# Vasilispapg/CVML-GoalNet

Hardware: AMD Instinct MI355X
Metric: training clips/sec at batch 64, 16-frame 224² clips; logit MAE vs CPU ref (higher is better)
Workload: dtype f32; 1 GPU; AVM train step (forward + broadcast-MSE + backward + fused Adam), 64 clips x 16 frames = 1024 frames of 3x224x224 + 30x30 MFCC per GPU; dropout live (device masks), BatchNorm train mode; frames_per_gpu=1024, h=224, w=224, parallelism=dp1, ddp_semantics=local BN + local MSE per rank, gradient mean (standard DDP), params=1286754369

## Files before the change

### cvml_goalnet_amd/_lib.py

```python
from __future__ import annotations

import ctypes
import os
from ctypes import c_char_p, c_double, c_float, c_int, c_int64, c_size_t, c_uint32, c_uint64, c_void_p

_HERE = os.path.dirname(os.path.abspath(__file__))
LIB_PATH = os.environ.get("GOALNET_LIB_PATH") or os.path.join(_HERE, "libgoalnet_hip.so")
ABI_VERSION = 7
STAT_PARTS = 1024
ADAM_RANGES_MAX = 32

P = c_void_p


class RowCopy(ctypes.Structure):
    _fields_ = [("src", c_void_p), ("dst", c_void_p), ("row_bytes", c_int64), ("nrows", c_int), ("gather", c_int), ("cursor", c_void_p),
                ("cursor_bias", c_int64)]


class AdamRange(ctypes.Structure):
    _fields_ = [("begin", c_int64), ("count", c_int64), ("skipped", c_int64)]


PROTOTYPES = {
# ... 55 lines not shown
    "goalnet_split_padded": (c_int, [c_int, P, P, P, P, P, c_int, c_int, c_int, c_int, P]),
    "goalnet_split_rows": (c_int, [c_int, P, c_int64, P, P, c_int, P, P, c_int64, c_int64, P]),
    "goalnet_conv3x3_fwd_split": (c_int, [c_int, P, P, P, c_int, P, c_int, c_int, c_int, c_int, c_int, P, P]),
    "goalnet_conv3x3_wgrad_split_ws_bytes": (c_size_t, [c_int, c_int, c_int, c_int, c_int, c_int]),
    "goalnet_conv3x3_wgrad_split": (c_int, [c_int, P, P, P, P, c_size_t, c_int, c_int, c_int, c_int, c_int, P, P]),
    "goalnet_linear_split_ok": (c_int, [c_int, c_int, c_int64, c_int]),
    "goalnet_linear_fwd_split_ws_bytes": (c_size_t, [c_int, c_int, c_int64, c_int]),
    "goalnet_linear_fwd_split": (c_int, [c_int, P, P, P, c_int, P, c_int64, P, c_int64, P, c_int64, c_int, c_int64, c_int, P, c_size_t, P, P]),
    "goalnet_linear_bwd_dx_split": (c_int, [c_int, P, P, P, c_int64, c_int, c_int64, c_int, P, P]),
    "goalnet_linear_bwd_dw_split": (c_int, [c_int, P, P, P, c_int, c_int64, c_int, P, P]),
    "goalnet_linear_bwd_dx_bf16": (c_int, [P, c_int64, P, P, c_int64, P, c_int64, c_int, c_int64, c_int, c_int, P]),
    "goalnet_linear_bwd_dx_bf16_o16_ok": (c_int, [c_int, c_int64, c_int]),
    "goalnet_linear_bwd_dx_bf16_o16": (c_int, [P, c_int64, P, P, c_int64, c_int, c_int64, c_int, c_int, P]),
    "goalnet_conv3x3_fwd_bf16p_o16_ok": (c_int, [c_int, c_int, c_int, c_int, c_int]),
    "goalnet_conv3x3_fwd_bf16p_o16": (c_int, [P, P, P, c_int, P, c_int, c_int, c_int, c_int, c_int, c_int, P]),
    "goalnet_linear_bwd_dw_bf16": (c_int, [P, c_int64, P, c_int64, P, c_int, c_int64, c_int, c_int, P]),
    "goalnet_linear_fwd_ws_bytes": (c_size_t, [c_int, c_int64, c_int]),
    "goalnet_linear_fwd": (c_int, [P, c_int64, P, P, c_int, P, P, c_int, P, c_int64, P, c_int64, P, c_int64,
                                   c_int, c_int64, c_int, P, c_size_t, P]),
    "goalnet_linear_bwd_dx": (c_int, [P, c_int64, P, P, c_int64, P, c_int64, c_int, c_int64, c_int, P]),
    "goalnet_linear_bwd_dw": (c_int, [P, c_int64, P, c_int64, P, P, c_int, P, P, c_int, c_int64, c_int, P]),
    "goalnet_linear_bwd_dw_adam": (c_int, [P, c_int64, P, c_int64, P, P, c_int, P, P, P, P, c_int, c_int64, c_int,
                                           c_double, c_double, c_double, c_double, P, c_int64, c_float, P]),
    "goalnet_colsum": (c_int, [P, c_int64, c_int, c_int, P, P]),
    "goalnet_mul": (c_int, [P, c_int64, P, c_int64, P, c_int64, c_int, c_int, P]),
    "goalnet_conv1d_fwd": (c_int, [P, P, P, c_int, P, c_int, c_int, c_int, c_int, c_int, c_int, P]),
    "goalnet_conv1d_bwd_ws_bytes": (c_size_t, [c_int, c_int, c_int]),
    "goalnet_conv1d_bwd": (c_int, [P, P, P, P, P, P, c_int, c_int, c_int, c_int, c_int, c_int, P, c_size_t, P]),
    "goalnet_conv1d_bwd_small": (c_int, [P, P, P, P, P, P, P, c_int, c_int, c_int, c_int, c_int, c_int, P]),
    "goalnet_relu_bwd": (c_int, [P, P, P, c_int64, P]),
    "goalnet_mlp_blocks": (c_int, []),
    "goalnet_mlp_fwd": (c_int, [P, c_int64, c_int, P, P, P, P, P, P, P, P, P, P, P, c_int, P, P]),
    "goalnet_mlp_bwd_ws_bytes": (c_size_t, [c_int]),
    "goalnet_mlp_bwd": (c_int, [P, P, P, c_int64, P, c_int64, P, P, P, P, c_int64, P, c_int, c_int, c_int, P, c_size_t, P, P]),
    "goalnet_head_fwd": (c_int, [P, c_int64, P, P, P, P, c_int, c_int, P]),
    "goalnet_head_bwd": (c_int, [P, P, P, c_int64, P, P, c_int64, P, c_int64, P, P, c_int, c_int, P]),
    "goalnet_mse_bcast": (c_int, [P, P, c_int, P, P, P]),
    "goalnet_cubic_resample": (c_int, [P, P, P, c_int64, c_int, c_int, P]),
    "goalnet_logmel_slots": (c_int, [P, P, P, c_int, c_int, P, P, P, P, P, P, P, P]),
    "goalnet_mfcc_from_logmel": (c_int, [P, P, c_int, c_int, P, P, P, P, c_int, c_int, c_double, P]),
    "goalnet_cls_head_fwd": (c_int, [P, c_int64, P, P, P, P, c_int, c_int, c_int, P]),
    "goalnet_cross_entropy": (c_int, [P, P, P, P, c_int, c_int, P]),
    "goalnet_cls_head_bwd": (c_int, [P, P, P, c_int64, P, P, c_int64, P, c_int64, P, P, c_int, c_int, c_int, P]),
    "goalnet_argmax_plus1": (c_int, [P, P, c_int, c_int, P]),
    "goalnet_adam_step": (c_int, [P, P, P, P, c_int64, c_double, c_double, c_double, c_double, c_int, c_float, P]),
    "goalnet_counter_add": (c_int, [P, c_int64, P]),
# ... 67 lines not shown
```

### cvml_goalnet_amd/avm.py

```python
from __future__ import annotations

import math
import os
from typing import List, Optional

import torch
import torch.nn as nn
from torch.nn.parameter import UninitializedParameter

from . import ops
from ._lib import GoalnetError
from .synth import BASE_SEED, DROP_P, TID_DROP

F32 = torch.float32
BN_EPS = 1e-5
BN_MOMENTUM = 0.1
_ALIGN = 64


class _LazyFlags:

    def requires_grad_(self, requires_grad: bool = True):
        for p in self.parameters():
            p.requires_grad = requires_grad
# ... 48 lines not shown
            return r, None
        ev = torch.cuda.Event()
        ev.record(self.side)
        return r, ev

    @staticmethod
    def wait(ev):
        if ev is not None:
            torch.cuda.current_stream().wait_event(ev)

    def join(self):
        if self.enabled and self.forked:
            torch.cuda.current_stream().wait_stream(self.side)
            self.forked = False
        self.keep.clear()


class _Bwd:

    def __init__(self, model, train, fork):
        self.model, self.train, self.fork = model, train, fork
        self.scratch = {}
        self.dbias = {}
        self.T = train.__contains__

    def any_T(self, *layers):
        return any(f"{layer}.{leaf}" in self.train for layer in layers for leaf in ("weight", "bias"))

    def G(self, name):
        m = self.model
        if name in self.train:
            return m._gflat(name)
        s = m.spec(name)
        if s.kind in ("ohwi", "lin5") and name != "visbl.conv1.weight":
            raise GoalnetError(f"a backward that does not train {name} asked for its gradient")
        t = self.scratch.get(name)
        if t is None:
            t = self.scratch[name] = torch.empty(s.numel, dtype=F32, device=m._device)
        return t


class _Spec:
    __slots__ = ("name", "kind", "shape", "numel", "offset", "fan_in")

    def __init__(self, name, kind, shape, fan_in):
        self.name, self.kind, self.shape, self.fan_in = name, kind, tuple(shape), fan_in
# ... 16 lines not shown
    return out


EPI_FUSE_MIN_ROWS = 256
EPI_FUSE_SKINNY_ROWS = 16


def epi_fuse_pieces(env):
    if env is None or env in ("", "1"):
        return frozenset("a")
    if env == "0":
        return frozenset()
    return frozenset(ch for ch in env.lower() if ch in "a")


def epi_fuse_dw_adam(n, *, plain, synced, precision, train_w5, shadowed, inspected, forced, pieces):
    if forced is False or "a" not in pieces:
        return False
    if inspected and forced is not True:
        return False
    if not (plain and not synced and precision == "fp32" and train_w5 and not shadowed):
        return False
    if n <= EPI_FUSE_SKINNY_ROWS:
        return False
    return forced is True or n >= EPI_FUSE_MIN_ROWS


class AVM(_LazyFlags, nn.Module):
    def __init__(self, audio_included, device=None, seed: Optional[int] = None, precision: str = "fp32", head: str = "regression",
                 num_classes: int = 5):
        super().__init__()
        self.audio_included = audio_included
        if head not in ("regression", "classifier"):
            raise ValueError("head must be 'regression' (the reference's live code) or 'classifier' (its commented-out variant)")
        if not 2 <= num_classes <= 8:
            raise ValueError("num_classes must be in 2..8")
        self.head = head
        self.num_classes = num_classes if head == "classifier" else 1
        if precision not in ("fp32", "bf16", "fp16", "bf16x6", "fp16x3"):
            raise ValueError("precision must be 'fp32' (the reference's arithmetic), 'bf16x6' / 'fp16x3' (fp32 operands as bf16 triples / scaled "
                             "fp16 pairs on the 16-bit MFMA: fp32-grade), 'bf16' or 'fp16' (16-bit MFMA contractions)")
        self._loss_scale, self._loss_scale_user = 1.0, False
        self._loss_scale_backoff = 0
        self._skipped_seen = 0
        self.precision = precision
        self._guard = None
# ... 30 lines not shown
        self._sat_out = {}
        self._bwd_frozen = frozenset()
        self._fp16_frozen = None
        self._arena_grad_scale = 1.0
        self._w5b, self._w5b_version = None, None
        self._load_count = 0
        self._state = None
        self._materialized = False
        self.grad_sync = None
        self.stat_sync = None
        self.grad_bf16 = os.environ.get("GOALNET_DZ16", "1") != "0"
        self.act_bf16 = os.environ.get("GOALNET_P16", "1") != "0"
        env = os.environ.get
        self.x6_off = env("GOALNET_X6_OFF") == "1"
        self.x6_linear5 = env("GOALNET_X6_LINEAR5", "1") != "0"
        self.x3_wgrad2 = env("GOALNET_X3_WGRAD2", "1") != "0"
        self.x3_dgrad2 = env("GOALNET_X3_DGRAD2", "1") != "0"
        self.mlp_fused = env("GOALNET_MLP_FUSED", "1") != "0"
        self.small_bn = env("GOALNET_SMALL_BN", "1") != "0"
        self.force_bf5 = env("GOALNET_FORCE_BF5") == "1"
        self.overlap_pair = env("GOALNET_OVERLAP_PAIR", "1") != "0"
        self.epi_fuse = None
        self.epi_fused_dw = 0
        self.keep_ctx = False
        self.last_ctx = None
        self.last_used_w5b = False
        self._side_stream = None
        self.overlap_rows = int(os.environ.get("GOALNET_OVERLAP_ROWS", "64"))
        _ol = os.environ.get("GOALNET_OVERLAP_LARGE")
        self.overlap_large = _ol == "1"
        self.overlap_auto = _ol is None
        self.time_labels = None
        self.kernel_events = None

    @property
    def precision(self) -> str:
        return self._precision

    @precision.setter
    def precision(self, value: str):
        if value not in ("fp32", "bf16", "fp16", "bf16x6", "fp16x3"):
            raise ValueError("precision must be 'fp32', 'bf16x6', 'fp16x3', 'bf16' or 'fp16'")
        self._precision = value
        self._half = value in ("bf16", "fp16")
        self._parts = {"bf16x6": 3, "fp16x3": 2}.get(value, 0)
        self._x6 = self._parts > 0
# ... 334 lines not shown
        return ops.split_padded(self._parts, x, scale, shift, self._padbuf(key, n, h, w, self._parts * c), n, h, w, c, amax=am), am

    def _split_mat(self, x2d, rows, c, scale=None, shift=None, bnC=0):
        am = self._amax_of(x2d, rows, c, scale=scale, shift=shift, bnC=bnC)
        return ops.split_rows(self._parts, x2d, torch.empty(rows * self._parts * c, dtype=self._h16, device=x2d.device), rows, c,
                              scale=scale, shift=shift, bnC=bnC, amax=am), am

    def _x6_linear5(self, n, k5):
        return self._x6 and ops.linear_split_ok(self._parts, n, k5, 512) and not self.x6_off and self.x6_linear5

    def _mlp_fused(self, n):
        return n <= 16 and self.head == "regression" and self.mlp_fused

    def _bf5(self, n):
        return self._half and (n > 16 or self.force_bf5)

    def _pair(self, n):
        return self._large_overlap(n) and self.overlap_pair

    def _small_bn(self, a, b, n, hc, wc, c):
        return (a.dtype == F32 and b.dtype == F32 and self.stat_sync is None and c <= 512 and n * hc * wc * c <= ops.SMALL_BN_ELEMS
                and self.small_bn)

    def _bn_block(self, y, n, hc, wc, c, i, save, p16=False):
        dev = self._device
        assert p16 or y.dtype == F32
        p = torch.empty(n, hc - 2, wc - 2, c, dtype=self._h16 if p16 else F32, device=dev)
        idx = torch.empty(n, hc - 2, wc - 2, c, dtype=torch.uint8, device=dev) if save else None
        bn = getattr(self.visbl, f"bnorm{i}")
        st = torch.empty(4, c, dtype=F32, device=dev)
        count = n * (hc - 2) * (wc - 2)
        if not self.training:
            ops.pool_bn_eval_fwd(y, p, idx, self._pflat(f"visbl.bnorm{i}.weight"), self._pflat(f"visbl.bnorm{i}.bias"),
                                 bn.running_mean, bn.running_var, BN_EPS, st, n, hc, wc, c)
            return p, idx, st
        if self._small_bn(y, p, n, hc, wc, c):
            ops.pool_bn_fwd_small(y, p, idx, self._pflat(f"visbl.bnorm{i}.weight"), self._pflat(f"visbl.bnorm{i}.bias"),
                                  bn.running_mean, bn.running_var, BN_MOMENTUM, BN_EPS, st, n, hc, wc, c)
            bn.num_batches_tracked += 1
            return p, idx, st
        partials = torch.empty(ops.stat_parts(8 * n) * 2 * c, dtype=torch.float64, device=dev)
        ops.pool_bnstats_fwd(y, p, idx, partials, n, hc, wc, c)
        if self.stat_sync is not None:
            partials, count = self._global_sums(partials, 2 * c), count * self.stat_sync.world
        ops.bn_finalize(partials, self._pflat(f"visbl.bnorm{i}.weight"), self._pflat(f"visbl.bnorm{i}.bias"),
                        bn.running_mean, bn.running_var, BN_MOMENTUM, BN_EPS, count, c,
# ... 125 lines not shown
            x = hs[4]
        for li, (key, width) in enumerate(() if fused_mlp else (("0", 512), ("3", 512), ("6", 256), ("9", 128))):
            hnext = torch.empty(n, width, dtype=F32, device=dev)
            m = torch.empty(n, width, dtype=F32, device=dev) if save else None
            ops.linear_fwd(x, P(f"fusion.{key}.weight"), P(f"fusion.{key}.bias"), hnext, relu=True,
                           dropmask=masks[1 + li], mult_out=m)
            hs.append(hnext); ms.append(m)
            x = hnext
        if self.head == "classifier":
            logit = torch.empty(n, self.num_classes, dtype=F32, device=dev)
            out = torch.empty(n, self.num_classes, dtype=F32, device=dev)
            ops.cls_head_fwd(x, P("fusion.12.weight"), P("fusion.12.bias"), logit, out)
        elif not fused_mlp:
            logit = torch.empty(n, dtype=F32, device=dev)
            out = torch.empty(n, dtype=F32, device=dev)
            ops.head_fwd(x, P("fusion.12.weight"), P("fusion.12.bias"), logit, out)
        if save:
            ctx.update(p1=p1, idx1=idx1, st1=st1, p2=p2, idx2=idx2, st2=st2, p3=p3, idx3=idx3, st3=st3,
                       a1=a1, a2=a2, hs=hs, ms=ms, logit=logit, out=out, l1=l1, l2=l2)
        self.last_logit = logit
        self.last_features = cat
        return out, ctx

    def _block_bwd(self, bwd, dbn, ctx, i, n, hc, wc, c):
        dev, G, bias = self._device, bwd.G, bwd.T(f"visbl.conv{i}.bias")
        p, idx, st = ctx[f"p{i}"], ctx[f"idx{i}"], ctx[f"st{i}"]
        npix = n * (hc - 2) * (wc - 2)
        small = self._small_bn(dbn, p, n, hc, wc, c) and not (self._half and i > 1)
        frozen = ctx["eval"]
        if small:
            coef3 = torch.empty(3 * c, dtype=F32, device=dev)
            (ops.bn_bwd_reduce_small_eval if frozen else ops.bn_bwd_reduce_small)(
                dbn, p, st[0], st[1], self._pflat(f"visbl.bnorm{i}.weight"), G(f"visbl.bnorm{i}.weight"), G(f"visbl.bnorm{i}.bias"),
                coef3, n, hc, wc, c)
            dy = torch.empty(n, hc, wc, c, dtype=F32, device=dev)
            dparts = torch.empty(ops.stat_parts(8 * n) * c, dtype=torch.float64, device=dev)
            ops.bnpool_bwd(dbn, p, idx, coef3, dy, dparts, n, hc, wc, c)
            if i > 1 and bias:
                bwd.dbias[i] = (dparts, c)
            return dy
        coef3 = torch.empty(3 * c, dtype=F32, device=dev)
        partials = torch.empty(ops.stat_parts(npix // 64) * 2 * c, dtype=torch.float64, device=dev)
        ops.bn_bwd_reduce(dbn, p, st[0], st[1], partials, npix, c)
        if frozen:
            ops.bn_bwd_finalize_eval(partials, self._pflat(f"visbl.bnorm{i}.weight"), st[1], c,
                                     G(f"visbl.bnorm{i}.weight"), G(f"visbl.bnorm{i}.bias"), coef3)
        else:
            ops.bn_bwd_finalize(partials, self._pflat(f"visbl.bnorm{i}.weight"), st[0], st[1], npix, c,
                                G(f"visbl.bnorm{i}.weight"), G(f"visbl.bnorm{i}.bias"), coef3)
        if self.stat_sync is not None and not frozen:
            scratch = torch.empty(2 * c, dtype=F32, device=dev)
            ops.bn_bwd_finalize(self._global_sums(partials, 2 * c), self._pflat(f"visbl.bnorm{i}.weight"), st[0], st[1],
                                npix * self.stat_sync.world, c, scratch[:c], scratch[c:], coef3)
        dparts = torch.empty(ops.stat_parts(8 * n) * c, dtype=torch.float64, device=dev)
        if self._half and i > 1 and self._bwd16_ok(wc):
            dy = self._padbuf(f"dy{i}", n, hc, wc, c)
            ops.bnpool_bwd_bf16p(dbn, p, idx, coef3, None, dy, dparts, n, hc, wc, c)
        elif self._half and i > 1:
            dy32 = torch.empty(n, hc, wc, c, dtype=F32, device=dev)
            ops.bnpool_bwd(dbn, p, idx, coef3, dy32, dparts, n, hc, wc, c)
            dy = ops.to_bf16_padded(dy32, None, None, self._padbuf(f"dy{i}", n, hc, wc, c), n, hc, wc, c)
        else:
            dy = torch.empty(n, hc, wc, c, dtype=F32, device=dev)
            ops.bnpool_bwd(dbn, p, idx, coef3, dy, dparts, n, hc, wc, c)
        if not bias:
            return dy
        if i == 1:
            ops.partials_sum(dparts, ops.stat_parts(8 * n), c, c, G(f"visbl.conv{i}.bias"))
        else:
            bwd.fork.run(lambda: ops.partials_sum(dparts, ops.stat_parts(8 * n), c, c, G(f"visbl.conv{i}.bias")), dparts)
        return dy

    def _conv_block_bwd(self, bwd, i, dbn, ctx, n, hc, wc, cin, cout, wt, flipped, wait_ev, pair, out16, split_dgrad, after_block=None,
                        dgrad=True):
        dev, P, G, fork = self._device, self._pflat, bwd.G, bwd.fork
        wname, xs = f"visbl.conv{i}.weight", f"x{i - 1}s"
        flops = 2.0 * n * hc * wc * 9 * cin * cout
        dy = self._block_bwd(bwd, dbn, ctx, i, n, hc, wc, cout)
        if after_block:
            after_block()
        split = not self._half and xs in ctx
        if not bwd.T(wname):
            wg = None
            if split and split_dgrad and dgrad:
                dys, ady = self._split_act(f"dy{i}s", dy, None, None, n, hc, wc, cout)
        elif self._half:
            wg, keep = (ops.conv3x3_wgrad_bf16, ctx[f"xh{i - 1}"], dy, G(wname), n, hc, wc, cin, cout), (dy,)
        elif split:
            dys, ady = self._split_act(f"dy{i}s", dy, None, None, n, hc, wc, cout)
            osc_w = self._osc(ady, ctx[xs + "_amax"])
            wg, keep = (ops.conv3x3_wgrad_split, self._parts, ctx[xs], dys, G(wname), n, hc, wc, cin, cout, osc_w), (dys, osc_w)
        else:
            st_in = ctx[f"st{i - 1}"]
            wg, keep = (ops.conv3x3_wgrad, ctx[f"p{i - 1}"], st_in[2], st_in[3], dy, G(wname), n, hc, wc, cin, cout), (dy,)

        def wgrad():
            if wg is not None:
                fork.run(lambda: self._timed("conv_wgrad", flops, *wg), *keep)
        if not pair:
            wgrad()
        if not dgrad:
            if pair:
                wgrad()
            return None
        if flipped:
            fork.wait(wait_ev)
        else:
            ops.conv3x3_weight_flip(P(wname), wt, cout, cin)
        o16 = out16 and ops.conv3x3_fwd_bf16p_o16_ok(n, hc, wc, cout, cin)
        dx = torch.empty(n, hc, wc, cin, dtype=self._h16 if o16 else F32, device=dev)
        if self._half:
            wtb = ops.cast_bf16(wt, torch.empty(wt.shape, dtype=self._h16, device=dev))
            self._timed("conv_dgrad", flops, ops.conv3x3_fwd_bf16p_o16 if o16 else ops.conv3x3_fwd_bf16p,
                        dy, wtb, None, False, dx, n, hc, wc, cout, cin)
        elif split and split_dgrad:
            wts, awt = self._split_w(wt, cin * 9, cout)
            self._timed("conv_dgrad", flops, ops.conv3x3_fwd_split, self._parts,
                        dys, wts, None, False, dx, n, hc, wc, cout, cin, self._osc(ady, awt))
        else:
            self._timed("conv_dgrad", flops, ops.conv3x3_fwd, dy, None, None, wt, None, False, dx, n, hc, wc, cout, cin)
        if pair:
            wgrad()
        return dx

    def backward_device(self, ctx, dout, on_bucket=None, after_linear5=None, inputs=None, params=True, reduce=0, frozen=None,
                        fused_w5=None):
        need_aud, need_vis = inputs if inputs is not None else (False, False)
        need_aud = need_aud and self.audio_included
        train = frozenset()
        if params:
            frozen = self._frozen_names() if frozen is None else frozenset(frozen)
            self._check_freeze(frozen)
            train = frozenset(s.name for s in self._specs) - frozen
        if self._half and ctx["padgen"] != (self._padgen["x1"], self._padgen["x2"]):
            raise RuntimeError("precision='bf16': a second training-mode forward overwrote the saved bf16 operands before "
                               "backward ran; call backward after each forward (as the reference's loop does)")
        for i in (3, 2):
            xs = f"x{i - 1}s"
            if not self._half and xs in ctx and f"visbl.conv{i}.weight" in train and ctx[xs + "_gen"] != self._padgen[xs]:
                raise RuntimeError(f"precision='{self.precision}': a second training-mode forward overwrote the saved split operands "
                                   "before backward ran; call backward after each forward (as the reference's loop does)")
# ... 105 lines not shown
                dz5b = ops.cast_bf16(dz5.contiguous(), torch.empty(n, 512, dtype=self._h16, device=dev))
                if train_w5:
                    fork.run(lambda: ops.linear_bwd_dw_bf16(dz5b, ctx["xh3"].view(n, k5), G("visbl.linear5.weight")), dz5b)
                bucket_done(1)
                if not need_b3:
                    pass
                elif o16_3:
                    ops.linear_bwd_dx_bf16_o16(dz5b, ctx["w5b"], dbn3.view(n, k5))
                else:
                    ops.linear_bwd_dx_bf16(dz5b, ctx["w5b"], dbn3.view(n, k5), mult=None)
            elif "x3s" in ctx:
                dz5s, adz = self._split_mat(dz5, n, 512)
                if train_w5:
                    osc_w = self._osc(adz, ctx["x3s_amax"])
                    fork.run(lambda: ops.linear_bwd_dw_split(self._parts, dz5s, ctx["x3s"], G("visbl.linear5.weight"), n, k5, 512, oscale=osc_w), dz5s, osc_w)
                bucket_done(1)
                if need_b3:
                    ops.linear_bwd_dx_split(self._parts, dz5s, ctx["w5s"], dbn3.view(n, k5), n, k5, 512, oscale=self._osc(adz, ctx["w5s_amax"]))
            else:
                fuse5 = fused_w5 is not None and train_w5
                if train_w5 and not fuse5:
                    fork.run(lambda: ops.linear_bwd_dw(dz5, p3f, G("visbl.linear5.weight"), scale=st3[2], shift=st3[3], bnC=512), dz)
                bucket_done(1)
                if need_b3:
                    ops.linear_bwd_dx(dz5, P("visbl.linear5.weight"), dbn3.view(n, k5), mult=None)
                if fuse5:
                    fused_w5(dz5, p3f, st3[2], st3[3])
            linear5_done()
        else:
            bucket_done(1)

        b2, b3 = (hp1, wp1, 64, 256), (hp2, wp2, 256, 512)
        dbn2 = dbn1 = None
        if dbn3 is not None:
            dbn2 = self._conv_block_bwd(bwd, 3, dbn3, ctx, n, *b3, wt3, flips_early, flips_ev, pair, out16=dz16 and self._bwd16_ok(wp1),
                                        split_dgrad=True, after_block=lambda: [cb(fork) for cb in deferred_l5], dgrad=need_b2)
        del dbn3
        if dbn2 is not None:
            dbn1 = self._conv_block_bwd(bwd, 2, dbn2, ctx, n, *b2, wt2, flips_early, None, pair, out16=False,
                                        split_dgrad=self.x3_dgrad2, dgrad=need_b1)
        del dbn2

        if dbn1 is not None:
            train_c1 = any_T("visbl.conv1")
            dy1 = self._block_bwd(bwd, dbn1, ctx, 1, n, h1, w1, 64)
            if train_c1:
                ops.conv1_wgrad(ctx["visual"], dy1, G("visbl.conv1.weight"), G("visbl.conv1.bias"), n, h, w)
# ... 315 lines not shown
```

### cvml_goalnet_amd/csrc/gemm_f32.hip

```cpp
#include <stdlib.h>

#include "adam.h"
#include "gemm_common.h"
#include "skinny.h"

using namespace goalnet;

namespace {

constexpr int BM = 128, BN = 128, BK = 32;
constexpr int LDR = 128;
constexpr int OP_FLOATS = BM * BK;

__device__ __forceinline__ int kc_off(int row, int chunk) { return row * BK + ((chunk ^ ((row >> 1) & 7)) << 2); }

__device__ __forceinline__ float4 f4zero() { return make_float4(0.f, 0.f, 0.f, 0.f); }
__device__ __forceinline__ float4 f4fma(float4 v, float4 s, float4 t) {
    return make_float4(fmaf(v.x, s.x, t.x), fmaf(v.y, s.y, t.y), fmaf(v.z, s.z, t.z), fmaf(v.w, s.w, t.w));
}

typedef unsigned int u32x4 __attribute__((ext_vector_type(4)));
constexpr unsigned OOB = 0xFFFFFF00u;

__device__ __forceinline__ float4 f4sel(bool v, float4 a) { return v ? a : f4zero(); }
// ... 739 lines not shown
    s.step_size = wave_uniform(s.step_size); s.bc2_sqrt = wave_uniform(s.bc2_sqrt);
    s.b2 = wave_uniform(s.b2); s.omb1 = wave_uniform(s.omb1); s.omb2 = wave_uniform(s.omb2);
    const int lane = tid & 63, wave = tid >> 6;
    const int wm = wave >> 1, wn = wave & 1;
    const int r = lane & 31, h = lane >> 5;
    f32x16 acc[2][2];
    gemm_mainloop<AL, BL, STAGES>(ap, bp, tm, tn, 0, ktiles, tid, acc);
    adam_acc(ae, s, rows, cols, ld, acc, tm, tn, wm, wn, r, h);
}

template <class AL, class BL, int EPI>
int launch_gemm_epi(const char* name, const typename AL::P& ap, const typename BL::P& bp, const AdamEpi& ae, int64_t M, int64_t N,
                    int64_t ld, int ktiles, int m_fast, hipStream_t st) {
    const int64_t tiles_m = (M + BM - 1) / BM, tiles_n = (N + BN - 1) / BN;
    GN_REQUIRE(tiles_m * tiles_n < (1ll << 31), GOALNET_E_SHAPE, "%s: too many tiles", name);
    static const int force_stages = getenv("GOALNET_F32_STAGES") ? atoi(getenv("GOALNET_F32_STAGES")) : 0;
    const dim3 grid((unsigned)(tiles_m * tiles_n), 1, 1);
    if (force_stages == 1 || (force_stages != 2 && AL::ONE_STAGE))
        hipLaunchKernelGGL((gemm_f32_epi_kernel<AL, BL, 1, EPI>), grid, dim3(256), 0, st, ap, bp, ae, (int)M, (int)N, ld, (int)tiles_m,
                           (int)tiles_n, m_fast, ktiles);
    else
        hipLaunchKernelGGL((gemm_f32_epi_kernel<AL, BL, 2, EPI>), grid, dim3(256), 0, st, ap, bp, ae, (int)M, (int)N, ld, (int)tiles_m,
                           (int)tiles_n, m_fast, ktiles);
    GN_LAUNCH_CHECK(name);
    return 0;
}

__global__ __launch_bounds__(256) void splitk_reduce_kernel(const float* slabs, int nsplit, int64_t slab_stride, EpiP ep) {
    const int c4n = ep.cols >> 2;
    const int64_t total = (int64_t)ep.rows * c4n;
    for (int64_t i = (int64_t)blockIdx.x * blockDim.x + threadIdx.x; i < total; i += (int64_t)gridDim.x * blockDim.x) {
        const int64_t row = i / c4n;
        const int col = (int)(i - row * c4n) * 4;
        const float* s = slabs + row * ep.cols + col;
        float4 a = *reinterpret_cast<const float4*>(s);
        for (int k = 1; k < nsplit; ++k) {
            const float4 b = *reinterpret_cast<const float4*>(s + (int64_t)k * slab_stride);
            a.x += b.x; a.y += b.y; a.z += b.z; a.w += b.w;
        }
        if (ep.oscale) { const int k = *ep.oscale; a.x = ldexpf(a.x, k); a.y = ldexpf(a.y, k); a.z = ldexpf(a.z, k); a.w = ldexpf(a.w, k); }
        if (ep.corr_u) {
            const int tap = col / ep.corr_C, ci = col - tap * ep.corr_C;
            const float u = ep.corr_u[row * 9 + tap];
            const float4 shv = *reinterpret_cast<const float4*>(ep.corr_sh + ci);
            a.x = fmaf(-shv.x, u, a.x); a.y = fmaf(-shv.y, u, a.y); a.z = fmaf(-shv.z, u, a.z); a.w = fmaf(-shv.w, u, a.w);
        }
// ... 400 lines not shown
                               float grad_scale, void* stream) {
    GN_REQUIRE(dy && x && p && m && v && step, GOALNET_E_NULL, "linear_bwd_dw_adam: null pointer");
    GN_REQUIRE((scale == nullptr) == (shift == nullptr), GOALNET_E_NULL, "linear_bwd_dw_adam: scale/shift must both be set or both NULL");
    GN_REQUIRE(M > 0 && J > 0 && K > 0 && K < (1ll << 31) - 256, GOALNET_E_SHAPE, "linear_bwd_dw_adam: bad dims");
    GN_REQUIRE(J % 4 == 0 && K % 4 == 0, GOALNET_E_SHAPE, "linear_bwd_dw_adam: J and K must be multiples of 4");
    GN_REQUIRE(!scale || (bnC > 0 && bnC % 4 == 0), GOALNET_E_SHAPE, "linear_bwd_dw_adam: bnC must be a positive multiple of 4");
    GN_REQUIRE(M > SKINNY_MAX_M, GOALNET_E_SHAPE, "linear_bwd_dw_adam: M=%d is served by the weight-streaming kernels (M > %d here)", M, SKINNY_MAX_M);
    GN_REQUIRE(aligned16(dy) && aligned16(x) && aligned16(scale) && aligned16(shift) && lddy % 4 == 0 && ldx % 4 == 0,
               GOALNET_E_ALIGN, "linear_bwd_dw_adam: pointers / leading dims must be 16-byte aligned");
    GN_REQUIRE(aligned16(p) && aligned16(m) && aligned16(v), GOALNET_E_ALIGN, "linear_bwd_dw_adam: p, m and v must be 16-byte aligned");
    hipStream_t st = (hipStream_t)stream;
    if (db) { const int rc = goalnet_colsum(dy, lddy, M, J, db, stream); if (rc) return rc; }
    const int ktiles = (M + BK - 1) / BK;
    MCLoader<false>::P ap{dy, lddy, J, M, nullptr, nullptr, 1};
    const AdamEpi ae{p, m, v, lr, beta1, beta2, (float)eps, grad_scale, step, step_bias};
    if (scale) {
        MCLoader<true>::P bp{x, ldx, (int)K, M, scale, shift, bnC};
        return launch_gemm_epi<MCLoader<false>, MCLoader<true>, EPIK_ADAM>("linear_bwd_dw_adam", ap, bp, ae, J, K, K, ktiles, 1, st);
    }
    MCLoader<false>::P bp{x, ldx, (int)K, M, nullptr, nullptr, 1};
    return launch_gemm_epi<MCLoader<false>, MCLoader<false>, EPIK_ADAM>("linear_bwd_dw_adam", ap, bp, ae, J, K, K, ktiles, 1, st);
}

}
```

### cvml_goalnet_amd/ops.py

```python
from __future__ import annotations

import ctypes
import os

import torch

from . import _lib
from ._lib import STAT_PARTS, check

F32 = torch.float32


def _s():
    return torch.cuda.current_stream().cuda_stream


def _p(t):
    return 0 if t is None else t.data_ptr()


def _chk(*ts):
    for t in ts:
        if t is None:
            continue
# ... 551 lines not shown

def linear_fwd(x, w, bias, y, *, relu=False, scale=None, shift=None, bnC=0, dropmask=None, mult_out=None, K=None):
    _chk(x, w, bias, y, scale, shift, dropmask, mult_out)
    M = x.shape[0]
    K = x.shape[1] if K is None else K
    J = y.shape[1]
    _req(w.numel() == J * K and y.shape[0] == M, "linear_fwd: argument check failed: w.numel() == J * K and y.shape[0] == M")
    nbytes = lib().goalnet_linear_fwd_ws_bytes(M, K, J)
    ws = torch.empty(max(nbytes // 4, 1), dtype=F32, device=x.device) if nbytes else None
    check(lib().goalnet_linear_fwd(x.data_ptr(), _ld(x), _p(scale), _p(shift), bnC, w.data_ptr(), _p(bias), int(relu),
                                   _p(dropmask), 0 if dropmask is None else _ld(dropmask), y.data_ptr(), _ld(y),
                                   _p(mult_out), 0 if mult_out is None else _ld(mult_out), M, K, J, _p(ws), nbytes, _s()),
          "linear_fwd")
    return y


def linear_bwd_dx(dy, w, dx, mult=None):
    _chk(dy, w, dx, mult)
    M, J = dy.shape
    K = dx.shape[1]
    _req(w.numel() == J * K and dx.shape[0] == M, "linear_bwd_dx: argument check failed: w.numel() == J * K and dx.shape[0] == M")
    check(lib().goalnet_linear_bwd_dx(dy.data_ptr(), _ld(dy), w.data_ptr(), _p(mult), 0 if mult is None else _ld(mult),
                                      dx.data_ptr(), _ld(dx), M, K, J, _s()), "linear_bwd_dx")
    return dx


def linear_bwd_dw(dy, x, dw, *, scale=None, shift=None, bnC=0, db=None):
    _chk(dy, x, dw, scale, shift, db)
    M, J = dy.shape
    K = x.shape[1]
    _req(dw.numel() == J * K and x.shape[0] == M and (db is None or db.numel() == J), "linear_bwd_dw: argument check failed: dw.numel() == J * K and x.shape[0] == M and (db is None or db.numel() == J)")
    check(lib().goalnet_linear_bwd_dw(dy.data_ptr(), _ld(dy), x.data_ptr(), _ld(x), _p(scale), _p(shift), bnC, dw.data_ptr(), _p(db),
                                      M, K, J, _s()), "linear_bwd_dw")
    return dw


def linear_bwd_dw_adam(dy, x, p, m, v, lr, beta1, beta2, eps, step, *, scale=None, shift=None, bnC=0, db=None, grad_scale=1.0, step_bias=0):
    _chk(dy, x, p, m, v, scale, shift, db)
    M, J = dy.shape
    K = x.shape[1]
    _req(p.numel() == J * K and m.numel() == J * K and v.numel() == J * K and x.shape[0] == M and (db is None or db.numel() == J),
         "linear_bwd_dw_adam: argument check failed: p.numel() == m.numel() == v.numel() == J * K and x.shape[0] == M and (db is None or db.numel() == J)")
    _req(p.is_contiguous() and m.is_contiguous() and v.is_contiguous(), "linear_bwd_dw_adam: p, m and v must be contiguous")
    check(lib().goalnet_linear_bwd_dw_adam(dy.data_ptr(), _ld(dy), x.data_ptr(), _ld(x), _p(scale), _p(shift), bnC, p.data_ptr(), m.data_ptr(),
                                           v.data_ptr(), _p(db), M, K, J, lr, beta1, beta2, eps, _ctr(step), int(step_bias), grad_scale, _s()),
          "linear_bwd_dw_adam")
# ... 340 lines not shown
```

### include/goalnet_hip.h

```cpp
#ifndef GOALNET_HIP_H
#define GOALNET_HIP_H

#include <stddef.h>
#include <stdint.h>

#ifdef __cplusplus
extern "C" {
#endif

#define GOALNET_ABI_VERSION 7

#define GOALNET_OK 0
#define GOALNET_E_NULL (-1)
#define GOALNET_E_SHAPE (-2)
#define GOALNET_E_ALIGN (-3)
#define GOALNET_E_WORKSPACE (-4)

#define GOALNET_STAT_PARTS 1024
int goalnet_stat_parts(int64_t units);

int goalnet_abi_version(void);
const char* goalnet_last_error(void);

int goalnet_fill_uniform(float* dst, int64_t n, uint64_t seed, uint32_t tensor_id, float lo, float hi, void* stream);
// ... 111 lines not shown
int goalnet_linear_bwd_dx_bf16(const void* dy_bf16, int64_t lddy, const void* w_bf16, const float* mult, int64_t ldmult,
                               float* dx, int64_t lddx, int M, int64_t K, int J, int f16, void* stream);
int goalnet_linear_bwd_dx_bf16_o16_ok(int M, int64_t K, int J);
int goalnet_linear_bwd_dx_bf16_o16(const void* dy_bf16, int64_t lddy, const void* w_bf16, void* dx_bf16, int64_t lddx,
                                   int M, int64_t K, int J, int f16, void* stream);
int goalnet_linear_bwd_dw_bf16(const void* dy_bf16, int64_t lddy, const void* x_bf16, int64_t ldx, float* dw,
                               int M, int64_t K, int J, int f16, void* stream);

size_t goalnet_linear_fwd_ws_bytes(int M, int64_t K, int J);
int goalnet_linear_fwd(const float* x, int64_t ldx, const float* scale, const float* shift, int bnC,
                       const float* w, const float* bias, int relu, const float* dropmask, int64_t ldmask,
                       float* y, int64_t ldy, float* mult_out, int64_t ldmult,
                       int M, int64_t K, int J, void* ws, size_t ws_bytes, void* stream);
int goalnet_linear_bwd_dx(const float* dy, int64_t lddy, const float* w, const float* mult, int64_t ldmult,
                          float* dx, int64_t lddx, int M, int64_t K, int J, void* stream);
int goalnet_linear_bwd_dw(const float* dy, int64_t lddy, const float* x, int64_t ldx,
                          const float* scale, const float* shift, int bnC,
                          float* dw, float* db, int M, int64_t K, int J, void* stream);
int goalnet_linear_bwd_dw_adam(const float* dy, int64_t lddy, const float* x, int64_t ldx,
                               const float* scale, const float* shift, int bnC,
                               float* p, float* m, float* v, float* db, int M, int64_t K, int J,
                               double lr, double beta1, double beta2, double eps, const int64_t* step, int64_t step_bias,
                               float grad_scale, void* stream);
int goalnet_colsum(const float* x, int64_t ldx, int M, int J, float* out, void* stream);
int goalnet_mul(const float* x, int64_t ldx, const float* mult, int64_t ldmult, float* y, int64_t ldy,
                int M, int J, void* stream);

int goalnet_conv1d_fwd(const float* x, const float* w, const float* b, int relu, float* y,
                       int N, int Cin, int L, int Cout, int stride, int pad, void* stream);
size_t goalnet_conv1d_bwd_ws_bytes(int N, int Cin, int Cout);
int goalnet_conv1d_bwd(const float* x, const float* dz, const float* w, float* dx, float* dw, float* db,
                       int N, int Cin, int L, int Cout, int stride, int pad, void* ws, size_t ws_bytes, void* stream);
int goalnet_conv1d_bwd_small(const float* x, const float* dz, const float* y, const float* w, float* dx, float* dw, float* db,
                             int N, int Cin, int L, int Cout, int stride, int pad, void* stream);
int goalnet_relu_bwd(const float* dy, const float* y, float* dz, int64_t n, void* stream);

int goalnet_mlp_blocks(void);
int goalnet_mlp_fwd(const float* cat, int64_t ldcat, int K0, const float* const* w, const float* const* b,
                    const float* const* mask, const int64_t* ldmask, float* const* h, float* const* mult,
                    float* logit, float* out, const float* labels, float* loss, float* dout, int n, int* sync, void* stream);
size_t goalnet_mlp_bwd_ws_bytes(int n);
int goalnet_mlp_bwd(const float* dout, const float* out, const float* const* x, int64_t ldcat, const float* const* m, int64_t ldmcat,
                    const float* const* w, float* const* dw, float* const* db, float* dcat, int64_t lddcat, float* db5, int voff,
                    int n, int K0, void* ws, size_t ws_bytes, int* sync, void* stream);

int goalnet_head_fwd(const float* h, int64_t ldh, const float* w, const float* b, float* logit, float* out,
// ... 103 lines not shown
```

Measured before the change: 160.6 clips/s.

## Fuse BatchNorm backward reductions into conv dgrad and linear dx GEMM epilogues

Adds GEMM epilogues to the fp32 conv3x3 data-gradient and linear5 dx kernels that accumulate the per-channel BatchNorm backward sums (sum of dy and of dy times x-hat) in double while the output tile is written. A small fold kernel then reduces the per-tile sums into the stat partials. The next block's backward reuses these partials and skips its separate bn_bwd_reduce pass over the gradient and activations. The cost is extra reads of the saved activations inside the epilogue, an fp64 reduction through shared memory, and a workspace allocation on every call.

```diff
diff --git a/cvml_goalnet_amd/_lib.py b/cvml_goalnet_amd/_lib.py
--- a/cvml_goalnet_amd/_lib.py
+++ b/cvml_goalnet_amd/_lib.py
@@ -101,6 +101,11 @@
     "goalnet_linear_bwd_dw": (c_int, [P, c_int64, P, c_int64, P, P, c_int, P, P, c_int, c_int64, c_int, P]),
     "goalnet_linear_bwd_dw_adam": (c_int, [P, c_int64, P, c_int64, P, P, c_int, P, P, P, P, c_int, c_int64, c_int,
                                            c_double, c_double, c_double, c_double, P, c_int64, c_float, P]),
+    "goalnet_linear_bwd_dx_bnsums_ws_bytes": (c_size_t, [c_int, c_int64, c_int]),
+    "goalnet_linear_bwd_dx_bnsums": (c_int, [P, c_int64, P, P, c_int64, P, c_int64, P, P, c_int, P, c_size_t, P, c_int,
+                                             c_int, c_int64, c_int, P]),
+    "goalnet_conv3x3_dgrad_bnsums_ws_bytes": (c_size_t, [c_int, c_int, c_int, c_int, c_int]),
+    "goalnet_conv3x3_dgrad_bnsums": (c_int, [P, P, P, P, P, P, P, c_size_t, P, c_int, c_int, c_int, c_int, c_int, c_int, P]),
     "goalnet_colsum": (c_int, [P, c_int64, c_int, c_int, P, P]),
     "goalnet_mul": (c_int, [P, c_int64, P, c_int64, P, c_int64, c_int, c_int, P]),
     "goalnet_conv1d_fwd": (c_int, [P, P, P, c_int, P, c_int, c_int, c_int, c_int, c_int, c_int, P]),
diff --git a/cvml_goalnet_amd/avm.py b/cvml_goalnet_amd/avm.py
--- a/cvml_goalnet_amd/avm.py
+++ b/cvml_goalnet_amd/avm.py
@@ -94,6 +94,7 @@
         self.model, self.train, self.fork = model, train, fork
         self.scratch = {}
         self.dbias = {}
+        self.bn_parts = {}
         self.T = train.__contains__
 
     def any_T(self, *layers):
@@ -156,6 +157,22 @@
     if not (plain and not synced and precision == "fp32" and train_w5 and not shadowed):
         return False
     if n <= EPI_FUSE_SKINNY_ROWS:
+        return False
+    return forced is True or n >= EPI_FUSE_MIN_ROWS
+
+
+def epi_bn_pieces(env):
+    if env is None or env in ("", "1"):
+        return frozenset("bc")
+    if env == "0":
+        return frozenset()
+    return frozenset(ch for ch in env.lower() if ch in "bc")
+
+
+def epi_bn_sums(n, *, piece, precision, small_bn, ws_bytes, forced, pieces):
+    if forced is False or piece not in pieces:
+        return False
+    if precision != "fp32" or small_bn or not ws_bytes:
         return False
     return forced is True or n >= EPI_FUSE_MIN_ROWS
 
@@ -232,6 +249,9 @@
         self.overlap_pair = env("GOALNET_OVERLAP_PAIR", "1") != "0"
         self.epi_fuse = None
         self.epi_fused_dw = 0
+        self.epi_bn = None
+        self.epi_bn_b = 0
+        self.epi_bn_c = 0
         self.keep_ctx = False
         self.last_ctx = None
         self.last_used_w5b = False
@@ -612,6 +632,10 @@
         return (a.dtype == F32 and b.dtype == F32 and self.stat_sync is None and c <= 512 and n * hc * wc * c <= ops.SMALL_BN_ELEMS
                 and self.small_bn)
 
+    def _epi_bn(self, piece, n, small, ws_bytes):
+        return epi_bn_sums(n, piece=piece, precision=self.precision, small_bn=small, ws_bytes=ws_bytes, forced=self.epi_bn,
+                           pieces=epi_bn_pieces(os.environ.get("GOALNET_F32_EPI_BN")))
+
     def _bn_block(self, y, n, hc, wc, c, i, save, p16=False):
         dev = self._device
         assert p16 or y.dtype == F32
@@ -783,12 +807,13 @@
         self.last_features = cat
         return out, ctx
 
-    def _block_bwd(self, bwd, dbn, ctx, i, n, hc, wc, c):
+    def _block_bwd(self, bwd, dbn, ctx, i, n, hc, wc, c, partials=None):
         dev, G, bias = self._device, bwd.G, bwd.T(f"visbl.conv{i}.bias")
         p, idx, st = ctx[f"p{i}"], ctx[f"idx{i}"], ctx[f"st{i}"]
         npix = n * (hc - 2) * (wc - 2)
         small = self._small_bn(dbn, p, n, hc, wc, c) and not (self._half and i > 1)
         frozen = ctx["eval"]
+        assert partials is None or not small, "pre-filled partial rows belong to the large BatchNorm path"
         if small:
             coef3 = torch.empty(3 * c, dtype=F32, device=dev)
             (ops.bn_bwd_reduce_small_eval if frozen else ops.bn_bwd_reduce_small)(
@@ -801,8 +826,9 @@
                 bwd.dbias[i] = (dparts, c)
             return dy
         coef3 = torch.empty(3 * c, dtype=F32, device=dev)
-        partials = torch.empty(ops.stat_parts(npix // 64) * 2 * c, dtype=torch.float64, device=dev)
-        ops.bn_bwd_reduce(dbn, p, st[0], st[1], partials, npix, c)
+        if partials is None:
+            partials = torch.empty(ops.stat_parts(npix // 64) * 2 * c, dtype=torch.float64, device=dev)
+            ops.bn_bwd_reduce(dbn, p, st[0], st[1], partials, npix, c)
         if frozen:
             ops.bn_bwd_finalize_eval(partials, self._pflat(f"visbl.bnorm{i}.weight"), st[1], c,
                                      G(f"visbl.bnorm{i}.weight"), G(f"visbl.bnorm{i}.bias"), coef3)
@@ -837,7 +863,7 @@
         dev, P, G, fork = self._device, self._pflat, bwd.G, bwd.fork
         wname, xs = f"visbl.conv{i}.weight", f"x{i - 1}s"
         flops = 2.0 * n * hc * wc * 9 * cin * cout
-        dy = self._block_bwd(bwd, dbn, ctx, i, n, hc, wc, cout)
+        dy = self._block_bwd(bwd, dbn, ctx, i, n, hc, wc, cout, partials=bwd.bn_parts.pop(i, None))
         if after_block:
             after_block()
         split = not self._half and xs in ctx
@@ -878,6 +904,14 @@
             wts, awt = self._split_w(wt, cin * 9, cout)
             self._timed("conv_dgrad", flops, ops.conv3x3_fwd_split, self._parts,
                         dys, wts, None, False, dx, n, hc, wc, cout, cin, self._osc(ady, awt))
+        elif self._epi_bn("c", n, self._small_bn(dx, ctx[f"p{i - 1}"], n, hc + 2, wc + 2, cin),
+                          ops.conv3x3_dgrad_bnsums_ws_bytes(n, hc, wc, cout, cin)):
+            st_in = ctx[f"st{i - 1}"]
+            parts = torch.empty(ops.stat_parts(n * hc * wc // 64) * 2 * cin, dtype=torch.float64, device=dev)
+            self._timed("conv_dgrad", flops, ops.conv3x3_dgrad_bnsums, dy, wt, dx, ctx[f"p{i - 1}"], st_in[0], st_in[1], parts,
+                        n, hc, wc, cout, cin)
+            bwd.bn_parts[i - 1] = parts
+            self.epi_bn_c += 1
         else:
             self._timed("conv_dgrad", flops, ops.conv3x3_fwd, dy, None, None, wt, None, False, dx, n, hc, wc, cout, cin)
         if pair:
@@ -1029,7 +1063,13 @@
                 if train_w5 and not fuse5:
                     fork.run(lambda: ops.linear_bwd_dw(dz5, p3f, G("visbl.linear5.weight"), scale=st3[2], shift=st3[3], bnC=512), dz)
                 bucket_done(1)
-                if need_b3:
+                if need_b3 and self._epi_bn("b", n, self._small_bn(dbn3, ctx["p3"], n, hp2, wp2, 512),
+                                            ops.linear_bwd_dx_bnsums_ws_bytes(n, k5, 512)):
+                    parts = torch.empty(ops.stat_parts(n * hp3 * wp3 // 64) * 2 * 512, dtype=torch.float64, device=dev)
+                    ops.linear_bwd_dx_bnsums(dz5, P("visbl.linear5.weight"), dbn3.view(n, k5), p3f, st3[0], st3[1], 512, parts)
+                    bwd.bn_parts[3] = parts
+                    self.epi_bn_b += 1
+                elif need_b3:
                     ops.linear_bwd_dx(dz5, P("visbl.linear5.weight"), dbn3.view(n, k5), mult=None)
                 if fuse5:
                     fused_w5(dz5, p3f, st3[2], st3[3])
diff --git a/cvml_goalnet_amd/csrc/gemm_f32.hip b/cvml_goalnet_amd/csrc/gemm_f32.hip
--- a/cvml_goalnet_amd/csrc/gemm_f32.hip
+++ b/cvml_goalnet_amd/csrc/gemm_f32.hip
@@ -785,6 +785,160 @@
     else
         hipLaunchKernelGGL((gemm_f32_epi_kernel<AL, BL, 2, EPI>), grid, dim3(256), 0, st, ap, bp, ae, (int)M, (int)N, ld, (int)tiles_m,
                            (int)tiles_n, m_fast, ktiles);
+    GN_LAUNCH_CHECK(name);
+    return 0;
+}
+
+struct BnSumsEpi {
+    float* out; int64_t ld;
+    const float* p; int64_t ldp;
+    const float* mean; const float* invstd; int bnC;
+    double* ws;
+};
+
+template <bool BIL>
+__device__ __forceinline__ void bnsums_acc(const BnSumsEpi& be, int rows, int cols, const f32x16 (&acc)[2][2], int tm, int tn,
+                                           int wm, int wn, int r, int h, int tid, double* red) {
+    int col[2];
+    bool colok[2];
+    float mu[2], is[2];
+#pragma unroll
+    for (int fn = 0; fn < 2; ++fn) {
+        col[fn] = tn * GEMM_BN + wn * 64 + (BIL ? 2 * r + fn : fn * 32 + r);
+        colok[fn] = col[fn] < cols;
+        const int c = (colok[fn] ? col[fn] : 0) % be.bnC;
+        mu[fn] = be.mean[c];
+        is[fn] = be.invstd[c];
+    }
+    double s[2] = {0.0, 0.0}, q[2] = {0.0, 0.0};
+#pragma unroll
+    for (int fm = 0; fm < 2; ++fm) {
+        const int row0 = tm * GEMM_BM + wm * 64 + fm * 32 + 4 * h;
+#pragma unroll
+        for (int eb = 0; eb < 2; ++eb) {
+            float pv[8][2];
+#pragma unroll
+            for (int k = 0; k < 8; ++k) {
+                const int e = 8 * eb + k;
+                const int row = row0 + (e & 3) + 8 * (e >> 2);
+                const bool rok = row < rows;
+                if constexpr (BIL) {
+                    const bool ok = rok && colok[0];
+                    const float2 t = *reinterpret_cast<const float2*>(be.p + (ok ? (int64_t)row * be.ldp + col[0] : 0));
+                    pv[k][0] = t.x; pv[k][1] = t.y;
+                    if (ok) *reinterpret_cast<float2*>(be.out + (int64_t)row * be.ld + col[0]) = make_float2(acc[fm][0][e], acc[fm][1][e]);
+                } else {
+#pragma unroll
+                    for (int fn = 0; fn < 2; ++fn) {
+                        const bool ok = rok && colok[fn];
+                        pv[k][fn] = be.p[ok ? (int64_t)row * be.ldp + col[fn] : 0];
+                        if (ok) be.out[(int64_t)row * be.ld + col[fn]] = acc[fm][fn][e];
+                    }
+                }
+            }
+#pragma unroll
+            for (int k = 0; k < 8; ++k) {
+                const int e = 8 * eb + k;
+                const bool rok = row0 + (e & 3) + 8 * (e >> 2) < rows;
+#pragma unroll
+                for (int fn = 0; fn < 2; ++fn) {
+                    const bool ok = rok && colok[fn];
+                    const float d = ok ? acc[fm][fn][e] : 0.f;
+                    const float xh = ok ? (pv[k][fn] - mu[fn]) * is[fn] : 0.f;
+                    s[fn] += (double)d;
+                    q[fn] += (double)d * (double)xh;
+                }
+            }
+        }
+    }
+#pragma unroll
+    for (int fn = 0; fn < 2; ++fn) {
+        red[(2 * fn) * 256 + tid] = s[fn];
+        red[(2 * fn + 1) * 256 + tid] = q[fn];
+    }
+    __syncthreads();
+    if (tid < GEMM_BN) {
+        const int cwn = tid >> 6, w = tid & 63;
+        const int fn = BIL ? (w & 1) : (w >> 5), cr = BIL ? (w >> 1) : (w & 31);
+        double ss = 0.0, qq = 0.0;
+#pragma unroll
+        for (int cwm = 0; cwm < 2; ++cwm)
+#pragma unroll
+            for (int ch = 0; ch < 2; ++ch) {
+                const int t = (cwm * 2 + cwn) * 64 + ch * 32 + cr;
+                ss += red[(2 * fn) * 256 + t];
+                qq += red[(2 * fn + 1) * 256 + t];
+            }
+        const int c = tn * GEMM_BN + tid;
+        if (c < cols) *reinterpret_cast<double2*>(be.ws + ((int64_t)tm * cols + c) * 2) = make_double2(ss, qq);
+    }
+}
+
+template <class AL, class BL, int STAGES>
+__global__ __launch_bounds__(256, STAGES == 1 ? AL::ONE_STAGE_BLOCKS : 2) void gemm_f32_bnsums_kernel(typename AL::P ap, typename BL::P bp, BnSumsEpi be,
+                                                          int rows, int cols, int tiles_m, int tiles_n, int m_fast, int ktiles) {
+    static_assert(AL::KC, "the BatchNorm-sums epilogue: rows of the output are the A operand's rows in MFMA order");
+    const int tid = threadIdx.x;
+    int tm, tn;
+    tile_of_block(tiles_m, tiles_n, m_fast, tm, tn);
+    const int lane = tid & 63, wave = tid >> 6;
+    const int wm = wave >> 1, wn = wave & 1;
+    const int r = lane & 31, h = lane >> 5;
+    f32x16 acc[2][2];
+    if constexpr (AL::STRIP) {
+        static_assert(STAGES == 1 && BL::KC, "the strip form: one B stage");
+        __shared__ __attribute__((aligned(16))) float lstrip[STRIP_FLOATS];
+        __shared__ __attribute__((aligned(16))) float lbs[OP_FLOATS];
+        AL al(ap, tm * BM, tid);
+        BL bl(bp, tn * BN, tid);
+#pragma unroll
+        for (int i = 0; i < 2; ++i)
+#pragma unroll
+            for (int j = 0; j < 2; ++j)
+#pragma unroll
+                for (int e = 0; e < 16; ++e) acc[i][j][e] = 0.f;
+        conv_strip_loop(al, bl, lstrip, lbs, acc, ktiles, tid, wn, r, h);
+        static_assert(OP_FLOATS * sizeof(float) >= 1024 * sizeof(double), "the B stage holds the sums");
+        bnsums_acc<!BL::KC>(be, rows, cols, acc, tm, tn, wm, wn, r, h, tid, reinterpret_cast<double*>(lbs));
+    } else {
+        __shared__ double red[1024];
+        gemm_mainloop<AL, BL, STAGES>(ap, bp, tm, tn, 0, ktiles, tid, acc);
+        bnsums_acc<!BL::KC>(be, rows, cols, acc, tm, tn, wm, wn, r, h, tid, red);
+    }
+}
+
+__global__ __launch_bounds__(256) void bnsums_fold_kernel(const double* __restrict__ ws, int64_t units, int C, double* __restrict__ partials,
+                                                         int nparts) {
+    const int c = blockIdx.y * 256 + threadIdx.x;
+    if (c >= C) return;
+    const int j = blockIdx.x;
+    const double2* w2 = reinterpret_cast<const double2*>(ws);
+    double s0 = 0.0, q0 = 0.0, s1 = 0.0, q1 = 0.0;
+    int64_t u = j;
+    for (; u + nparts < units; u += 2 * (int64_t)nparts) {
+        const double2 a = w2[u * C + c], b = w2[(u + nparts) * C + c];
+        s0 += a.x; q0 += a.y;
+        s1 += b.x; q1 += b.y;
+    }
+    if (u < units) {
+        const double2 a = w2[u * C + c];
+        s0 += a.x; q0 += a.y;
+    }
+    partials[(int64_t)j * 2 * C + c] = s0 + s1;
+    partials[(int64_t)j * 2 * C + C + c] = q0 + q1;
+}
+
+template <class AL, class BL>
+int launch_gemm_bnsums(const char* name, const typename AL::P& ap, const typename BL::P& bp, const BnSumsEpi& be, int64_t M, int64_t N,
+                       int ktiles, int m_fast, double* partials, int nparts, hipStream_t st) {
+    const int64_t tiles_m = (M + BM - 1) / BM, tiles_n = (N + BN - 1) / BN;
+    GN_REQUIRE(tiles_m * tiles_n < (1ll << 31), GOALNET_E_SHAPE, "%s: too many tiles", name);
+    const dim3 grid((unsigned)(tiles_m * tiles_n), 1, 1);
+    hipLaunchKernelGGL((gemm_f32_bnsums_kernel<AL, BL, AL::STRIP ? 1 : 2>), grid, dim3(256), 0, st, ap, bp, be, (int)M, (int)N, (int)tiles_m,
+                       (int)tiles_n, m_fast, ktiles);
+    GN_LAUNCH_CHECK(name);
+    hipLaunchKernelGGL(bnsums_fold_kernel, dim3((unsigned)nparts, (unsigned)((be.bnC + 255) / 256)), dim3(256), 0, st, be.ws,
+                       tiles_m * (N / be.bnC), be.bnC, partials, nparts);
     GN_LAUNCH_CHECK(name);
     return 0;
 }
@@ -1231,4 +1385,59 @@
     return launch_gemm_epi<MCLoader<false>, MCLoader<false>, EPIK_ADAM>("linear_bwd_dw_adam", ap, bp, ae, J, K, K, ktiles, 1, st);
 }
 
-}
+size_t goalnet_linear_bwd_dx_bnsums_ws_bytes(int M, int64_t K, int J) {
+    if (M <= SKINNY_MAX_M || K <= 0 || J <= 0) return 0;
+    return (size_t)((M + BM - 1) / BM) * (size_t)K * 2 * sizeof(double);
+}
+
+int goalnet_linear_bwd_dx_bnsums(const float* dy, int64_t lddy, const float* w, float* dx, int64_t lddx,
+                                 const float* p, int64_t ldp, const float* mean, const float* invstd, int bnC,
+                                 void* ws, size_t ws_bytes, double* partials, int nparts, int M, int64_t K, int J, void* stream) {
+    GN_REQUIRE(dy && w && dx && p && mean && invstd && ws && partials, GOALNET_E_NULL, "linear_bwd_dx_bnsums: null pointer");
+    GN_REQUIRE(M > 0 && J > 0 && K > 0 && K < (1ll << 31) - 256, GOALNET_E_SHAPE, "linear_bwd_dx_bnsums: bad dims");
+    GN_REQUIRE(J % BK == 0, GOALNET_E_SHAPE, "linear_bwd_dx_bnsums: J=%d must be a multiple of %d", J, BK);
+    GN_REQUIRE(bnC > 0 && bnC % 4 == 0 && K % bnC == 0, GOALNET_E_SHAPE, "linear_bwd_dx_bnsums: bnC=%d must be a multiple of 4 that divides K", bnC);
+    GN_REQUIRE(M > SKINNY_MAX_M, GOALNET_E_SHAPE, "linear_bwd_dx_bnsums: M=%d is served by the weight-streaming kernels (M > %d here)", M, SKINNY_MAX_M);
+    GN_REQUIRE(nparts >= 1 && nparts <= GOALNET_STAT_PARTS, GOALNET_E_SHAPE, "linear_bwd_dx_bnsums: nparts=%d must be in [1, %d]", nparts, GOALNET_STAT_PARTS);
+    GN_REQUIRE(lddx >= K && ldp >= K, GOALNET_E_SHAPE, "linear_bwd_dx_bnsums: leading dims of dx and p must be >= K");
+    GN_REQUIRE(aligned16(dy) && aligned16(w) && aligned16(dx) && aligned16(p) && aligned16(mean) && aligned16(invstd) && aligned16(ws) &&
+               aligned16(partials) && lddy % 4 == 0 && lddx % 4 == 0 && ldp % 4 == 0,
+               GOALNET_E_ALIGN, "linear_bwd_dx_bnsums: pointers / leading dims must be 16-byte aligned");
+    GN_REQUIRE(ws_bytes >= goalnet_linear_bwd_dx_bnsums_ws_bytes(M, K, J), GOALNET_E_WORKSPACE, "linear_bwd_dx_bnsums: workspace too small");
+    KCLoader<false>::P ap{dy, lddy, M, nullptr, nullptr, 1, 0};
+    MCLoader<false>::P bp{w, K, (int)K, J, nullptr, nullptr, 1};
+    const BnSumsEpi be{dx, lddx, p, ldp, mean, invstd, bnC, (double*)ws};
+    return launch_gemm_bnsums<KCLoader<false>, MCLoader<false>>("linear_bwd_dx_bnsums", ap, bp, be, M, K, J / BK, 1, partials, nparts, (hipStream_t)stream);
+}
+
+size_t goalnet_conv3x3_dgrad_bnsums_ws_bytes(int N, int H, int W, int Cin, int Cout) {
+    if (N <= 0 || H <= 0 || W <= 0 || Cin <= 0 || Cout <= 0 || Cin % BK || Cout % 4) return 0;
+    const int64_t M = (int64_t)N * H * W;
+    const bool narrow = Cout <= 64 && !getenv("GOALNET_F32_N64_OFF");
+    if (!conv_strip_f32(W, conv_splits_f32(M, Cin, Cout), narrow, false)) return 0;
+    return (size_t)((M + BM - 1) / BM) * (size_t)Cout * 2 * sizeof(double);
+}
+
+int goalnet_conv3x3_dgrad_bnsums(const float* dy, const float* w, float* dx, const float* p, const float* mean, const float* invstd,
+                                 void* ws, size_t ws_bytes, double* partials, int nparts, int N, int H, int W, int Cin, int Cout,
+                                 void* stream) {
+    GN_REQUIRE(dy && w && dx && p && mean && invstd && ws && partials, GOALNET_E_NULL, "conv3x3_dgrad_bnsums: null pointer");
+    GN_REQUIRE(N > 0 && H > 0 && W > 0 && Cin > 0 && Cout > 0, GOALNET_E_SHAPE, "conv3x3_dgrad_bnsums: non-positive dim");
+    GN_REQUIRE(Cin % BK == 0, GOALNET_E_SHAPE, "conv3x3_dgrad_bnsums: Cin=%d must be a multiple of %d", Cin, BK);
+    GN_REQUIRE(Cout % 4 == 0, GOALNET_E_SHAPE, "conv3x3_dgrad_bnsums: Cout=%d must be a multiple of 4", Cout);
+    const int64_t M = (int64_t)N * H * W;
+    GN_REQUIRE(M < (1ll << 31) - 256, GOALNET_E_SHAPE, "conv3x3_dgrad_bnsums: N*H*W too large");
+    GN_REQUIRE(nparts >= 1 && nparts <= GOALNET_STAT_PARTS, GOALNET_E_SHAPE, "conv3x3_dgrad_bnsums: nparts=%d must be in [1, %d]", nparts, GOALNET_STAT_PARTS);
+    const size_t need = goalnet_conv3x3_dgrad_bnsums_ws_bytes(N, H, W, Cin, Cout);
+    GN_REQUIRE(need > 0, GOALNET_E_SHAPE, "conv3x3_dgrad_bnsums: this call is not served by the strip loader (split-K, W > %d or a narrow output)", CONV_STRIP_MAX_W);
+    GN_REQUIRE(aligned16(dy) && aligned16(w) && aligned16(dx) && aligned16(p) && aligned16(mean) && aligned16(invstd) && aligned16(ws) &&
+               aligned16(partials), GOALNET_E_ALIGN, "conv3x3_dgrad_bnsums: pointers must be 16-byte aligned");
+    GN_REQUIRE(ws_bytes >= need, GOALNET_E_WORKSPACE, "conv3x3_dgrad_bnsums: workspace too small");
+    ConvAStripLoader<false>::P ap{dy, H, W, Cin, M, nullptr, nullptr};
+    KCLoader<false>::P bp{w, (int64_t)9 * Cin, Cout, nullptr, nullptr, 1, Cin};
+    const BnSumsEpi be{dx, Cout, p, Cout, mean, invstd, Cout, (double*)ws};
+    return launch_gemm_bnsums<ConvAStripLoader<false>, KCLoader<false>>("conv3x3_dgrad_bnsums", ap, bp, be, M, Cout, 9 * Cin / BK, 0, partials, nparts,
+                                                                        (hipStream_t)stream);
+}
+
+}
diff --git a/cvml_goalnet_amd/ops.py b/cvml_goalnet_amd/ops.py
--- a/cvml_goalnet_amd/ops.py
+++ b/cvml_goalnet_amd/ops.py
@@ -597,6 +597,45 @@
     _req(w.numel() == J * K and dx.shape[0] == M, "linear_bwd_dx: argument check failed: w.numel() == J * K and dx.shape[0] == M")
     check(lib().goalnet_linear_bwd_dx(dy.data_ptr(), _ld(dy), w.data_ptr(), _p(mult), 0 if mult is None else _ld(mult),
                                       dx.data_ptr(), _ld(dx), M, K, J, _s()), "linear_bwd_dx")
+    return dx
+
+
+def linear_bwd_dx_bnsums_ws_bytes(M, K, J):
+    return lib().goalnet_linear_bwd_dx_bnsums_ws_bytes(M, K, J)
+
+
+def linear_bwd_dx_bnsums(dy, w, dx, p, mean, invstd, bnC, partials):
+    _chk(dy, w, dx, p, mean, invstd, partials)
+    M, J = dy.shape
+    K = dx.shape[1]
+    _req(w.numel() == J * K and dx.shape[0] == M and tuple(p.shape) == (M, K), "linear_bwd_dx_bnsums: argument check failed: w.numel() == J * K and dx.shape[0] == M and p.shape == (M, K)")
+    _req(dy.dtype == F32 and w.dtype == F32 and dx.dtype == F32 and p.dtype == F32, "linear_bwd_dx_bnsums: fp32 dy, w, dx, p")
+    _req(mean.numel() == bnC and invstd.numel() == bnC, "linear_bwd_dx_bnsums: mean, invstd (bnC)")
+    nbytes = linear_bwd_dx_bnsums_ws_bytes(M, K, J)
+    _req(nbytes > 0, "linear_bwd_dx_bnsums: this call is not served (M <= 16); use linear_bwd_dx and bn_bwd_reduce")
+    ws = torch.empty(nbytes // 8, dtype=torch.float64, device=dx.device)
+    check(lib().goalnet_linear_bwd_dx_bnsums(dy.data_ptr(), _ld(dy), w.data_ptr(), dx.data_ptr(), _ld(dx), p.data_ptr(), _ld(p),
+                                             mean.data_ptr(), invstd.data_ptr(), bnC, ws.data_ptr(), nbytes, partials.data_ptr(),
+                                             _rows(partials, 2 * bnC), M, K, J, _s()), "linear_bwd_dx_bnsums")
+    return dx
+
+
+def conv3x3_dgrad_bnsums_ws_bytes(N, H, W, Cin, Cout):
+    return lib().goalnet_conv3x3_dgrad_bnsums_ws_bytes(N, H, W, Cin, Cout)
+
+
+def conv3x3_dgrad_bnsums(dy, w, dx, p, mean, invstd, partials, N, H, W, Cin, Cout):
+    _chk(dy, w, dx, p, mean, invstd, partials)
+    _req(dy.numel() == N * H * W * Cin and dx.numel() == p.numel() == N * H * W * Cout and w.numel() == Cout * 9 * Cin,
+         "conv3x3_dgrad_bnsums: argument check failed: dy.numel() == N * H * W * Cin and dx.numel() == p.numel() == N * H * W * Cout and w.numel() == Cout * 9 * Cin")
+    _req(dy.dtype == F32 and dx.dtype == F32 and p.dtype == F32 and dx.is_contiguous() and p.is_contiguous(), "conv3x3_dgrad_bnsums: contiguous fp32 dy, dx, p")
+    _req(mean.numel() == Cout and invstd.numel() == Cout, "conv3x3_dgrad_bnsums: mean, invstd (Cout)")
+    nbytes = conv3x3_dgrad_bnsums_ws_bytes(N, H, W, Cin, Cout)
+    _req(nbytes > 0, "conv3x3_dgrad_bnsums: this call is not served; use conv3x3_fwd and bn_bwd_reduce")
+    ws = torch.empty(nbytes // 8, dtype=torch.float64, device=dx.device)
+    check(lib().goalnet_conv3x3_dgrad_bnsums(dy.data_ptr(), w.data_ptr(), dx.data_ptr(), p.data_ptr(), mean.data_ptr(), invstd.data_ptr(),
+                                             ws.data_ptr(), nbytes, partials.data_ptr(), _rows(partials, 2 * Cout), N, H, W, Cin, Cout, _s()),
+          "conv3x3_dgrad_bnsums")
     return dx
 
 
diff --git a/include/goalnet_hip.h b/include/goalnet_hip.h
--- a/include/goalnet_hip.h
+++ b/include/goalnet_hip.h
@@ -157,6 +157,14 @@
                                float* p, float* m, float* v, float* db, int M, int64_t K, int J,
                                double lr, double beta1, double beta2, double eps, const int64_t* step, int64_t step_bias,
                                float grad_scale, void* stream);
+size_t goalnet_linear_bwd_dx_bnsums_ws_bytes(int M, int64_t K, int J);
+int goalnet_linear_bwd_dx_bnsums(const float* dy, int64_t lddy, const float* w, float* dx, int64_t lddx,
+                                 const float* p, int64_t ldp, const float* mean, const float* invstd, int bnC,
+                                 void* ws, size_t ws_bytes, double* partials, int nparts, int M, int64_t K, int J, void* stream);
+size_t goalnet_conv3x3_dgrad_bnsums_ws_bytes(int N, int H, int W, int Cin, int Cout);
+int goalnet_conv3x3_dgrad_bnsums(const float* dy, const float* w, float* dx, const float* p, const float* mean, const float* invstd,
+                                 void* ws, size_t ws_bytes, double* partials, int nparts, int N, int H, int W, int Cin, int Cout,
+                                 void* stream);
 int goalnet_colsum(const float* x, int64_t ldx, int M, int J, float* out, void* stream);
 int goalnet_mul(const float* x, int64_t ldx, const float* mult, int64_t ldmult, float* y, int64_t ldy,
                 int M, int J, void* stream);
```

Measured after the change: 161.7 clips/s, median of 6. Within noise of the previous version (+0.7%).
